# madsjulia/GeostatInversion.jl

Measured on AMD Instinct MI355X. Metric: randSVD GB/s + top-k singular-value rel-err, n=1e6 rank=256, higher is better.
Workload: dtype f64

## Files before the change

### geostatinversion.jl_amd/build.py

```python
import os
import shutil
import subprocess
import sys
from concurrent.futures import ThreadPoolExecutor

HERE = os.path.dirname(os.path.abspath(__file__))
CSRC = os.path.join(HERE, "csrc")
OBJ = os.path.join(HERE, "build")
LIB = os.path.join(HERE, "libgsi_hip.so")
SOURCES = ["gemm_f64.hip", "gemm_f64_gen1.hip", "syrk_f64.hip", "panel_lu_leaf.hip", "panel_lu_blocks.hip", "panel_lu_streamed.hip", "panel_lu_sharded.hip", "panel_qr.hip", "cholqr.hip", "lowrank_power.hip", "jacobi_svd.hip", "misc.hip", "lsqr_dev.hip", "block_cg.hip", "block_pcg.hip", "block_slq.hip", "pivoted_chol.hip", "pointcov_gemm.hip", "fft_cov.hip", "fft_gridcov_plan.hip", "fftrf_sample.hip", "fftrf_interp.hip", "interp_adjoint.hip", "gridcov_sample.hip","pcga_forward.hip", "fwd_adjoint.hip", "chol_saddle.hip", "posterior_var.hip",
           "hip_backend.hip", "hip_backend_products.hip", "hip_backend_sampler.hip", "hip_backend_panels.hip", "hip_backend_lowrank.hip", "hip_backend_pcga.hip",
           "hip_comm.hip", "pipeline.cpp", "solvers.cpp", "pcga.cpp", "api.cpp"]
HEADERS = ["backend.hpp", "hip_backend.hpp", "hip_backend_impl.hpp", "hip_common.hpp", "panel_lu_dev.hpp", "pipeline.hpp", "solvers.hpp", "pcga.hpp", "lsqr_state.hpp", "cg_state.hpp", "block_cg_host.hpp", "slq_state.hpp", "pchol_state.hpp", "pivoted_chol_host.hpp", "pointcov.hpp", "pointcov_gen.hpp", "host_staging.hpp", "gemm_f64_kernel.inc.hpp", "fft_line.hpp", "jacobi_sched.hpp", "fwd_plan.hpp", "fwd_adjoint_plan.hpp", "fwd_adjoint_host.hpp", "fftrf_points.hpp", "interp_adjoint_plan.hpp", "saddle_host.hpp", "posterior_host.hpp", "../../include/gsi_hip.h"]
CXXFLAGS = ["-O3", "-std=c++17", "-fPIC", "--offload-arch=gfx950", "-Wall", "-Wno-unused-function",
            "-Wno-unused-result", "-Wno-unused-value"]
RESOURCE_FLAG = "-Rpass-analysis=kernel-resource-usage"
_RES_KEYS = {"TotalSGPRs": "sgprs", "VGPRs": "vgprs", "AGPRs": "agprs", "ScratchSize [bytes/lane]": "scratch_bytes_per_lane",
             "Occupancy [waves/SIMD]": "occupancy_waves_per_simd", "SGPRs Spill": "sgpr_spills", "VGPRs Spill": "vgpr_spills",
             "LDS Size [bytes/block]": "lds_bytes_per_block", "Dynamic Stack": "dynamic_stack"}


def parse_resource_remarks(text):
    out, cur = {}, None
    for line in text.splitlines():
        if "remark:" not in line or "[-Rpass-analysis=kernel-resource-usage]" not in line:
            continue
        body = line.split("remark:", 1)[1].replace("[-Rpass-analysis=kernel-resource-usage]", "").strip()
        if ":" not in body:
            continue
        key, val = [x.strip() for x in body.rsplit(":", 1)]
        if key == "Function Name":
            cur = out.setdefault(val, {})
        elif cur is not None and key in _RES_KEYS:
            cur[_RES_KEYS[key]] = (val == "True") if key == "Dynamic Stack" else int(val)
    return out

# ... 82 lines not shown
```

### geostatinversion.jl_amd/context.py

```python
import ctypes as C

import numpy as np

from . import _lib as L


class Context:

    def __init__(self, device=0, lib=None):
        self.lib = lib or L.load()
        h = C.c_void_p()
        L.check(self.lib.gsi_ctx_create(C.byref(h), int(device)), self.lib)
        self.h = h
        self.device = int(device)
        self._children = []

    def close(self):
        if getattr(self, "h", None):
            for ch in list(self._children):
                ch.close()
            self.lib.gsi_ctx_destroy(self.h)
            self.h = None

    def __del__(self):
# ... 34 lines not shown
        row0 = min(r * pad, m)
        return row0, min(pad, m - row0)

    def profile(self, on=True):
        L.check(self.lib.gsi_ctx_profile(self.h, int(on)), self.lib)

    def phase_reset(self):
        L.check(self.lib.gsi_ctx_phase_reset(self.h), self.lib)

    def phase_times(self):
        ms = (C.c_double * len(L.PHASES))()
        cnt = (C.c_int64 * len(L.PHASES))()
        L.check(self.lib.gsi_ctx_phase_times(self.h, ms, cnt), self.lib)
        return {name: (ms[i], cnt[i]) for i, name in enumerate(L.PHASES)}

    def counters(self):
        out = (C.c_int64 * 4)()
        L.check(self.lib.gsi_ctx_counters(self.h, out), self.lib)
        return {"cholqr2": out[0], "householder": out[1], "jacobi_sweeps": out[2], "scholqr3": out[3]}

    LU_FORMS = ["none", "replicated", "per-step", "persistent-1hop", "persistent-2hop", "persistent-ov"]

    def path_info(self):
        n = 20
        out = (C.c_int64 * n)()
        L.check(self.lib.gsi_ctx_path_info(self.h, out, n), self.lib)
        forms = {self.LU_FORMS[f]: int(out[6 + f]) for f in range(1, 6) if out[6 + f]}
        return {"lu_form": self.LU_FORMS[out[0]] if 0 <= out[0] < 6 else int(out[0]), "lu_forms_run": forms,
                "lu_selftest_mask": int(out[1]), "collectives": int(out[2]), "n_ranks_seen": int(out[3]),
                "lu_timeouts": int(out[4]), "lu_timeouts_recovered": int(out[5]), "svd_sweep_cap_hits": int(out[12]),
                "lowrank_tails": int(out[13]), "lowrank_power_steps": int(out[14]), "lowrank_power_declines": int(out[15]),
                "lowrank_split_lus": int(out[16]), "lowrank_split_declines": int(out[17]),
                "lowrank_tail_overlaps": int(out[18]), "lowrank_tail_series_rounds": int(out[19])}

    def release_cache(self):
        L.check(self.lib.gsi_ctx_release_cache(self.h), self.lib)

    def device_bytes(self):
        b = C.c_int64()
        L.check(self.lib.gsi_ctx_device_bytes(self.h, C.byref(b)), self.lib)
        return b.value


class _Handle:
    _destroy = None

    def __init__(self, ctx, h):
        self.ctx, self.h = ctx, h
        ctx._children.append(self)

    def close(self):
        if getattr(self, "h", None):
            getattr(self.ctx.lib, self._destroy)(self.h)
            self.h = None
            if self in self.ctx._children:
                self.ctx._children.remove(self)
# ... 190 lines not shown
```

### geostatinversion.jl_amd/csrc/api.cpp

```cpp
#include <cmath>
#include <cstdlib>
#include <cstring>
#include <memory>
#include <new>
#include <string>
#include <vector>
#include "../../include/gsi_hip.h"
#include "pcga.hpp"
#include "solvers.hpp"
#include "pointcov.hpp"
#include "fftrf_points.hpp"
#include "cg_state.hpp"

using namespace gsi;

struct gsi_ctx {
  Context c;
};
struct gsi_op {
  Operator op;
};
struct gsi_mat {
  gsi_ctx* ctx;
  Buf buf;
// ... 178 lines not shown
  });
}

int gsi_ctx_path_info(gsi_ctx* ctx, int64_t* out, int64_t n_out) {
  return guarded([&] {
    REQUIRE(ctx && out && n_out >= 1, "bad argument");
    Context& c = ctx->c;
    int64_t v[GSI_PATH_INFO_COUNT] = {0};
    v[GSI_PATH_LU_FORM_LAST] = c.lu_form_last;
    v[GSI_PATH_LU_SELFTEST_MASK] = c.lus_mr_selftest;
    v[GSI_PATH_COLLECTIVES] = c.comm ? c.comm->ncollectives : 0;
    v[GSI_PATH_RANKS_SEEN] = c.ranks_seen;
    v[GSI_PATH_LU_TIMEOUTS] = c.be->lu_timeouts();
    v[GSI_PATH_LU_TIMEOUTS_RECOVERED] = c.lu_timeouts_recovered;
    for (int f = 0; f < (int)Context::LU_FORMS; ++f) v[GSI_PATH_LU_FORM_COUNTS + f] = c.lu_form_count[f];
    v[GSI_PATH_SVD_CAP_HITS] = c.be->svd_cap_hits();
    v[GSI_PATH_LOWRANK_TAILS] = c.lowrank_tails;
    v[GSI_PATH_LOWRANK_POWER_STEPS] = c.lowrank_power_steps;
    v[GSI_PATH_LOWRANK_POWER_DECLINES] = c.lowrank_power_declines;
    v[GSI_PATH_LOWRANK_SPLIT_LUS] = c.lowrank_split_lus;
    v[GSI_PATH_LOWRANK_SPLIT_DECLINES] = c.lowrank_split_declines;
    v[GSI_PATH_LOWRANK_TAIL_OVERLAPS] = c.be->lowrank_tail_overlaps();
    v[GSI_PATH_LOWRANK_TAIL_SERIES_ROUNDS] = c.be->lowrank_tail_series_rounds();
    for (int64_t i = 0; i < n_out; ++i) out[i] = i < GSI_PATH_INFO_COUNT ? v[i] : 0;
  });
}

int gsi_ctx_pinned_copy_rate(gsi_ctx* ctx, int64_t bytes, double* h2d_gbs, double* d2h_gbs) {
  return guarded([&] {
    REQUIRE(ctx && h2d_gbs && d2h_gbs, "NULL argument");
    REQUIRE(bytes >= 0 && bytes <= ((int64_t)64 << 30), "bad size");
    ctx->c.be->pinned_copy_rate(bytes, h2d_gbs, d2h_gbs);
  });
}

int gsi_ctx_rank(gsi_ctx* ctx, int* rank, int* nranks) {
  return guarded([&] {
    REQUIRE(ctx, "ctx is NULL");
    if (rank) *rank = ctx->c.rank();
    if (nranks) *nranks = ctx->c.nranks();
  });
}

int gsi_op_dense(gsi_ctx* ctx, gsi_op** op, const double* A_rows, int64_t m, int64_t n, int64_t lda,
                 int64_t row0, int64_t m_local) {
  return guarded([&] {
// ... 937 lines not shown
int gsi_gemm(gsi_ctx* ctx, int trans, int64_t m, int64_t l, int64_t k, double alpha, const double* A,
             int64_t lda, const double* B, int64_t ldb, double* C, int64_t ldc) {
  return guarded([&] {
    REQUIRE(ctx && A && B && C, "NULL argument");
    REQUIRE(m >= 1 && l >= 1 && k >= 1, "bad shape");
    const int64_t ar = trans ? k : m, ac = trans ? m : k;
    REQUIRE(lda >= ar && ldb >= k && ldc >= m, "leading dimension too small");
    Backend* be = ctx->c.be.get();
    Buf Ad(be, (size_t)ar * ac), Bd(be, (size_t)k * l), Cd(be, (size_t)m * l);
    be->upload2d(Ad.p, ar, A, lda, ar, ac);
    be->upload2d(Bd.p, k, B, ldb, k, l);
    if (trans) be->gemm_tn(m, l, k, alpha, Ad.p, ar, Bd.p, k, 0.0, Cd.p, m);
    else be->gemm_nn(m, l, k, alpha, Ad.p, ar, Bd.p, k, 0.0, Cd.p, m);
    be->download2d(C, ldc, Cd.p, m, m, l);
    check_async_errors(ctx->c);
  });
}

int gsi_gemm_view(gsi_ctx* ctx, int form, int trans, int64_t m, int64_t l, int64_t k, double alpha, double beta,
                  const double* A, int64_t lda, int64_t a_off, const double* B, int64_t ldb, int64_t b_off, double* C,
                  int64_t ldc, int64_t c_off, int64_t m_full, int64_t r0, int64_t* plan_out) {
  return guarded([&] {
    REQUIRE(ctx && A && C && plan_out, "NULL argument");
    REQUIRE(form >= 0 && form <= 3, "gemm_view: form is 0 (gemm), 1 (syrk upper), 2 (trmm upper) or 3 (NN row block)");
    REQUIRE(m >= 1 && l >= 1 && k >= 1, "bad shape");
    REQUIRE(form == 1 || B, "NULL argument");
    REQUIRE(form == 0 || (alpha == 1.0 && beta == 0.0), "gemm_view: forms 1 to 3 compute C = op(A) B (alpha 1, beta 0)");
    REQUIRE(form == 0 || !trans, "gemm_view: trans belongs to form 0");
    REQUIRE(form != 1 || m == l, "gemm_view: form 1 is the l x l product A'A (m == l)");
    REQUIRE(form != 3 || (r0 >= 0 && r0 + m <= m_full), "gemm_view: row block outside the full product");
    const bool tn = trans || form == 1;
    const int64_t ar = (form == 3) ? m_full : (tn ? k : m), ac = tn ? m : k;
    const int64_t crows = (form == 3) ? m_full : m;
    REQUIRE(lda >= ar && ldc >= crows && (form == 1 || ldb >= k), "leading dimension too small");
    REQUIRE(a_off >= 0 && b_off >= 0 && c_off >= 0, "negative offset");
    Backend* be = ctx->c.be.get();
    const size_t na = (size_t)a_off + (size_t)lda * (size_t)ac, nc = (size_t)c_off + (size_t)ldc * (size_t)l;
    const size_t nb = (form == 1) ? 1 : (size_t)b_off + (size_t)ldb * (size_t)l;
    Buf Ad(be, na), Bd(be, nb), Cd(be, nc);
    be->fill_bytes(Ad.p, 0xFF, na);
    be->fill_bytes(Bd.p, 0xFF, nb);
    be->upload2d(Ad.p + a_off, lda, A, ar, ar, ac);
    if (form != 1) be->upload2d(Bd.p + b_off, ldb, B, k, k, l);
    be->upload2d(Cd.p, (int64_t)nc, C, (int64_t)nc, (int64_t)nc, 1);
    be->gemm_view(form, trans != 0, m, l, k, alpha, Ad.p + a_off, lda, Bd.p + b_off, ldb, beta, Cd.p + c_off, ldc, m_full, r0,
                  plan_out);
    be->download2d(C, (int64_t)nc, Cd.p, (int64_t)nc, (int64_t)nc, 1);
    check_async_errors(ctx->c);
  });
}

// ... 699 lines not shown
```

### geostatinversion.jl_amd/csrc/backend.hpp

```cpp
#pragma once
#include <cstddef>
#include <cstdint>
#include <stdexcept>
#include <string>

namespace gsi {

struct Error : std::runtime_error {
  int code;
  Error(int c, const std::string& msg) : std::runtime_error(msg), code(c) {}
};

enum Phase : int {
  PH_GEMM_N = 0, PH_GEMM_T = 1, PH_LU = 2, PH_QR = 3, PH_SVD = 4, PH_SMALL_GEMM = 5,
  PH_COMM = 6, PH_OTHER = 7, PH_COMM_WAIT = 8, PH_COUNT = 9
};

struct FwdProduct {
  int64_t nobs = 0, n = 0, nnz = 0, nseg = 0, maxlen = 0;
  const int64_t* segptr = nullptr;
  const int64_t* rowseg = nullptr;
  const int32_t* colidx = nullptr;
  const double* vals = nullptr;
  const double* w = nullptr;
// ... 125 lines not shown
  virtual bool lus_mr_swaps_done() { return false; }
  virtual void lus_swap_pack(const double*, int64_t, int64_t, int64_t, int64_t, int64_t, int, double*) {}
  virtual void lus_swap_apply(double*, int64_t, int64_t, int64_t, int64_t, int64_t, int, const double*) {}
  virtual void qr_thinQ(double* Y, int64_t m, int64_t l, int64_t ld, double* R, bool replicated = false) = 0;
  virtual bool qr_thinQ_deferred(const double* Y, int64_t m, int64_t l, int64_t ld, const double** Q1, int64_t* ldq1,
                                 double* X2) { (void)Y; (void)m; (void)l; (void)ld; (void)Q1; (void)ldq1; (void)X2; return false; }
  virtual bool svd_tall_fused(const double*, int64_t, int64_t, int64_t, int64_t, double*, int64_t, double*, const double* Xr = nullptr) {
    (void)Xr;
    return false;
  }
  virtual bool sample_gram(const double* S, int64_t ld, int64_t n, int64_t N, double* G) {
    (void)S; (void)ld; (void)n; (void)N; (void)G;
    return false;
  }
  virtual bool lowrank_tail(const double* S, int64_t lds, int64_t n, int64_t N, const double* G, const double* T, int64_t l,
                            int64_t K, double c, double* Z, int64_t ldz, double* Sv, double* scratch = nullptr,
                            size_t scratch_doubles = 0) {
    (void)S; (void)lds; (void)n; (void)N; (void)G; (void)T; (void)l; (void)K; (void)c; (void)Z; (void)ldz; (void)Sv;
    (void)scratch; (void)scratch_doubles;
    return false;
  }
  virtual int64_t lowrank_tail_overlaps() { return 0; }
  virtual int64_t lowrank_tail_series_rounds() { return 0; }
  virtual void cq_gram_round_view(double* Gm, int64_t l, double* X, bool check, int32_t* out2, double* norm_out) {
    (void)Gm; (void)l; (void)X; (void)check; (void)out2; (void)norm_out;
    throw Error(1 , "cq_gram_round: not available on this backend");
  }
  virtual bool lowrank_power_step(const double* S, int64_t lds, int64_t n, int64_t N, const double* G, const double* T,
                                  const int32_t* ipiv, const double* L, int64_t ldl, int64_t l, double c, double* T_next) {
    (void)S; (void)lds; (void)n; (void)N; (void)G; (void)T; (void)ipiv; (void)L; (void)ldl; (void)l; (void)c; (void)T_next;
    return false;
  }
  virtual bool lowrank_split_ok(int64_t n, int64_t N, int64_t l, int64_t l1) {
    (void)n; (void)N; (void)l; (void)l1;
    return false;
  }
  virtual void lowrank_split_schur(const double* S, int64_t lds, int64_t n, int64_t N, const double* T, const int32_t* ipiv1,
                                   const double* P, int64_t ldp, int64_t l, int64_t l1, double c, double* Tt) {
    (void)S; (void)lds; (void)n; (void)N; (void)T; (void)ipiv1; (void)P; (void)ldp; (void)l; (void)l1; (void)c; (void)Tt;
    throw Error(1 , "lowrank_split_schur: not available on this backend");
  }
  virtual void lowrank_split_rows(double* P, int64_t ldp, int64_t n, int64_t l, int64_t l1) {
    (void)P; (void)ldp; (void)n; (void)l; (void)l1;
    throw Error(1 , "lowrank_split_rows: not available on this backend");
  }
  virtual void lowrank_split_join(double* P, int64_t ldp, int64_t n, int64_t l, int64_t l1, const int32_t* ipiv2,
// ... 228 lines not shown
```

### geostatinversion.jl_amd/csrc/hip_backend_impl.hpp

```cpp
#pragma once
#include <map>
#include <memory>
#include <mutex>
#include <set>
#include <string>
#include <vector>
#include "hip_backend.hpp"
#include "hip_common.hpp"
#include "host_staging.hpp"
#include "fftrf_points.hpp"

namespace gsi {

struct DevBuf {
  void* p = nullptr;
  size_t bytes = 0;
  bool pooled = false;
};

struct Carve {
  size_t total = 0;
  static constexpr size_t up8(size_t x) { return (x + 7) & ~(size_t)7; }
  size_t take(size_t count) { const size_t o = total; total += up8(count); return o; }
  size_t packed(size_t count) { const size_t o = total; total += count; return o; }
// ... 66 lines not shown
  void* upload2d_begin(double* dst, int64_t ldd, const double* host, int64_t ldh, int64_t rows, int64_t cols,
                       int64_t block_rows) override;
  void upload2d_wait_block(void* handle, int64_t b) override;
  void upload2d_end(void* handle) override;
  void pinned_copy_rate(int64_t bytes, double* h2d_gbs, double* d2h_gbs) override;
  void copy2d(double* dst, int64_t ldd, const double* src, int64_t lds, int64_t rows, int64_t cols) override;
  void fill_zero(double* p, size_t count) override;
  void fill_bytes(double* p, int byte, size_t count) override;
  void sync() override;
  void forgive_lost_coresidency() override;
  bool retryable_failure() override;
  int take_error(std::string* msg) override;
  void profile(bool on) override { prof_ = on; }
  void phase_begin(Phase p) override;
  void phase_end(Phase) override { phase_end_counted(true); }
  void phase_end_more(Phase) override { phase_end_counted(false); }
  void phase_reset() override;
  void phase_times(double* ms, int64_t* counts) override;
  void counters(int64_t* out4) override;
  int64_t lu_timeouts() override { return n_lu_timeouts_; }
  int64_t svd_cap_hits() override { return n_svd_cap_hits_; }
  int64_t lowrank_tail_overlaps() override { return n_tail_overlaps_; }
  int64_t lowrank_tail_series_rounds() override { return n_tail_series_rounds_; }
  void set_ranks_sharing_device(int n) override { ranks_sharing_device_ = n; }

  void gemm_nn(int64_t m, int64_t l, int64_t k, double alpha, const double* A, int64_t lda, const double* B,
               int64_t ldb, double beta, double* C, int64_t ldc) override;
  void gemm_nn_rowblock(int64_t m_full, int64_t r0, int64_t mb, int64_t l, int64_t k, const double* A, int64_t lda,
                        const double* B, int64_t ldb, double* C, int64_t ldc) override;
  void gemm_tn(int64_t m, int64_t l, int64_t k, double alpha, const double* A, int64_t lda, const double* B,
               int64_t ldb, double beta, double* C, int64_t ldc) override;
  void gemm_view(int form, bool trans, int64_t m, int64_t l, int64_t k, double alpha, const double* A, int64_t lda,
                 const double* B, int64_t ldb, double beta, double* C, int64_t ldc, int64_t m_full, int64_t r0,
                 int64_t* plan8) override;
  void gemm_nn_gridcov(int64_t m, int64_t l, int64_t k, const double* tab, int64_t nx, int64_t ny, int64_t roff,
                       int64_t koff, const double* B, int64_t ldb, double* C, int64_t ldc) override;
  void gemm_nn_pointcov(int64_t m, int64_t l, int64_t k, const double* pts, int d, int kind, double ell, double sigma2,
                        double nugget, int64_t roff, int64_t koff, const double* B, int64_t ldb, double* C,
                        int64_t ldc) override;
  void* fftcov_create(const int64_t N[3], double beta, int fftrf) override;
  void* fftcov_create_lags(const int64_t N[3], int kind, const double ell[3], double theta, double sigma2, double nugget,
                           const double* table, const double* table_mirror) override;
  void fftcov_destroy(void* plan) override;
  void fftcov_apply(void* plan, int64_t l, const double* X, int64_t ldx, double* Y, int64_t ldy) override;
  void center_rows(double* S, int64_t n, int64_t N, int64_t ld) override;
  void randn(double* p, size_t count, uint64_t seed) override;
// ... 123 lines not shown
                       double* x, bool* singular) override;
  int basis_quadform(const void* Z, int zbits, int64_t n, int64_t ldz, int64_t K, const double* W, int64_t ldw, int64_t ncols,
                     bool upper, const double* u, double* a, double* q, double* t) override;
  int scale_rows(int64_t m, int64_t c, const double* d, const double* src, int64_t lds, double* dst, int64_t ldd) override;

 private:
  void trim_pool(int64_t keep_bytes);
  void free_ws(DevBuf& b);
  void collect_garbage();
  void trim(DevBuf& b);
  void grow(DevBuf& b, size_t bytes);
  GemmWs gemm_ws(size_t doubles);
  HostStager* stager();
  static size_t stage_min_bytes();
  bool staged(bool h2d, double* dev, int64_t ldd, double* host, int64_t ldh, int64_t rows, int64_t cols);
  void drain_side() { if (st2_) (void)hipStreamSynchronize(st2_); }
  hipStream_t side_stream();
  int32_t read_flag(int slot);
  void check_launch(const char* what);
  void phase_end_counted(bool counted);
  hipEvent_t get_event();

  void fits_ws(const char* who, const char* form, size_t need, const GemmWs& ws, int64_t m, int64_t l, int64_t k);
  void gemm(const char* who, const GemmWs& ws, bool trans, int64_t m, int64_t l, int64_t k, double alpha, const double* A,
            int64_t lda, const double* B, int64_t ldb, double beta, double* C, int64_t ldc, hipk::GemmPlan* plan = nullptr);
  void gemm_rowblock(const char* who, const GemmWs& ws, int64_t m_full, int64_t r0, int64_t mb, int64_t l, int64_t k,
                     const double* A, int64_t lda, const double* B, int64_t ldb, double* C, int64_t ldc,
                     hipk::GemmPlan* plan = nullptr);
  void gemm_syrk_upper(const char* who, const GemmWs& ws, int64_t l, int64_t k, const double* A, int64_t lda, double* C,
                       int64_t ldc, hipk::GemmPlan* plan = nullptr);
  void gemm_trmm_upper(const char* who, const GemmWs& ws, int64_t m, int64_t l, int64_t k, const double* A, int64_t lda,
                       const double* B, int64_t ldb, double* C, int64_t ldc, hipk::GemmPlan* plan = nullptr);
  std::unique_ptr<FftCov> fftcov_new_plan(const int64_t N[3], int fftrf, bool* reembed, int* dims);
  void fft_rotate_apply(Scratch& buf, int64_t cur[3], int64_t& tot, int d, int64_t rows_out, int64_t period, FftFactor f);
  void fftcov_lags_to_spectrum(Scratch& bufh, int64_t cur[3], int64_t& tot, const FftCov* p, int d, bool sine);
  static size_t points_plan_doubles(const FftrfPointsPlan& plan);
  void upload_points_plan(const FftrfPointsPlan& plan, double* d);
  void interp_batch(const FftrfPointsPlan& plan, const double* dplan, const double* V, int64_t v_fs, int nb, double* dst,
                    int64_t ldd);
  void fftrf_batches(double* dst, int64_t ldd, int64_t row0, int64_t nloc, int64_t nf, int ndims, const int64_t* N, double k0,
                     double dk, double beta, const double* phi, int64_t ldphi, uint64_t seed, int64_t field0,
                     const FftrfPointsPlan* at);

  void lu_L_impl(double* Y, int64_t m, int64_t l, int64_t ld, int32_t* ipiv_host, int32_t** ipiv_dev_out);
  bool lu2_resident_ok() const;
  bool lu2_takes(int64_t m, hipk::Lu2Work* w);
// ... 16 lines not shown
  DevBuf ws_gemm_, ws_lu_, ws_split_, ws_qr_, ws_svd_, ws_blas2_, ws_lus_, ws_svdf_, ws_qr_hh_;
  DevBuf* const ws_all_[9] = {&ws_gemm_, &ws_lu_, &ws_split_, &ws_qr_, &ws_svd_, &ws_blas2_, &ws_lus_, &ws_svdf_, &ws_qr_hh_};
  std::mutex mu_;
  std::vector<DevBuf> sizes_;
  std::vector<DevBuf> pool_;
  std::vector<void*> garbage_;
  size_t garbage_bytes_ = 0;
  int64_t in_use_ = 0, pooled_ = 0;

  std::unique_ptr<HostStager> stager_;
  bool stager_failed_ = false;
  hipEvent_t ev_stage_ = nullptr;

  bool prof_ = false;
  Rec cur_{};
  std::vector<Rec> records_;
  std::vector<hipEvent_t> ev_pool_;
  double acc_ms_[PH_COUNT] = {0};
  int64_t acc_n_[PH_COUNT] = {0};
  int last_svd_sweeps_ = 0;
  int64_t n_svd_cap_hits_ = 0;
  int64_t n_cholqr_ = 0, n_householder_ = 0, n_scholqr3_ = 0;
  int64_t n_tail_overlaps_ = 0;
  int64_t n_tail_series_rounds_ = 0;

  std::map<std::pair<int64_t, bool>, int> skip_tier1_by_height_;

  std::map<int, int> lu2_resident_;
  bool lu2_lost_ = false, lu2_retry_ = false;
  int lu2_ov_resident_ = -1;

  int mr_force_ = 0;
  unsigned long long* mr_recs_ = nullptr;
  unsigned long long* mr_peer_[hipk::LU2_MAX_RANKS] = {nullptr};
  Comm* mr_comm_ = nullptr;
  uint32_t mr_epoch_ = 0;
  bool mr_disabled_ = false, mr_peer_swaps_ = true;
  bool mr_share_tried_ = false, mr_in_flight_ = false;
  int64_t mr_gen_ = 0, n_lu_timeouts_ = 0;
  std::string mr_reason_, mr_why_disabled_;
  std::set<int64_t> mr_warm_;
  hipk::Lu2MrWork mr_work_{};
  int64_t lus_part_col_ = -1, lus_part_mloc_ = 0;
  const double* lus_part_Y_ = nullptr;

  void* pin_power_ = nullptr;
// ... 4 lines not shown
```

### geostatinversion.jl_amd/csrc/hip_backend_products.hip

```cpp
#include <algorithm>
#include <cmath>
#include <cstdlib>
#include <cstring>
#include "hip_backend_impl.hpp"
#include "interp_adjoint_plan.hpp"

namespace gsi {

void HipBackend::fits_ws(const char* who, const char* form, size_t need, const GemmWs& ws, int64_t m, int64_t l, int64_t k) {
  if (need <= ws.doubles) return;
  throw Error(GSI_ERR_INTERNAL, std::string(who) + ": the " + form + " product " + std::to_string(m) + " x " + std::to_string(l) +
                                    " (K = " + std::to_string(k) + ") needs a workspace of " + std::to_string(need) +
                                    " doubles and was given " + std::to_string(ws.doubles));
}
void HipBackend::gemm(const char* who, const GemmWs& ws, bool trans, int64_t m, int64_t l, int64_t k, double alpha,
                      const double* A, int64_t lda, const double* B, int64_t ldb, double beta, double* C, int64_t ldc,
                      hipk::GemmPlan* plan) {
  fits_ws(who, trans ? "A'B" : "AB", hipk::gemm_workspace_doubles(m, l, k), ws, m, l, k);
  hipk::gemm_f64(st_, trans, m, l, k, alpha, A, lda, B, ldb, beta, C, ldc, ws.p, plan);
}
void HipBackend::gemm_rowblock(const char* who, const GemmWs& ws, int64_t m_full, int64_t r0, int64_t mb, int64_t l, int64_t k,
                               const double* A, int64_t lda, const double* B, int64_t ldb, double* C, int64_t ldc,
                               hipk::GemmPlan* plan) {
  fits_ws(who, "row-block", hipk::gemm_rowblock_workspace_doubles(m_full, mb, l, k), ws, mb, l, k);
  hipk::gemm_f64_nn_rowblock(st_, m_full, r0, mb, l, k, A, lda, B, ldb, C, ldc, ws.p, plan);
}
void HipBackend::gemm_syrk_upper(const char* who, const GemmWs& ws, int64_t l, int64_t k, const double* A, int64_t lda,
                                 double* C, int64_t ldc, hipk::GemmPlan* plan) {
  fits_ws(who, "A'A", hipk::gemm_syrk_workspace_doubles(l, k), ws, l, l, k);
  hipk::gemm_f64_syrk_upper(st_, l, k, A, lda, C, ldc, ws.p, plan);
}
void HipBackend::gemm_trmm_upper(const char* who, const GemmWs& ws, int64_t m, int64_t l, int64_t k, const double* A,
                                 int64_t lda, const double* B, int64_t ldb, double* C, int64_t ldc, hipk::GemmPlan* plan) {
  fits_ws(who, "A triu(B)", hipk::gemm_workspace_doubles(m, l, k), ws, m, l, k);
  hipk::gemm_f64_trmm_upper(st_, m, l, k, A, lda, B, ldb, C, ldc, ws.p, plan);
}

void HipBackend::gemm_nn(int64_t m, int64_t l, int64_t k, double alpha, const double* A, int64_t lda, const double* B,
                         int64_t ldb, double beta, double* C, int64_t ldc) {
  bind();
// ... 2 lines not shown
  check_launch("gemm_nn");
}
void HipBackend::gemm_nn_rowblock(int64_t m_full, int64_t r0, int64_t mb, int64_t l, int64_t k, const double* A, int64_t lda,
                                  const double* B, int64_t ldb, double* C, int64_t ldc) {
  bind();
  const GemmWs ws = gemm_ws(hipk::gemm_rowblock_workspace_doubles(m_full, mb, l, k));
  gemm_rowblock("gemm_nn_rowblock", ws, m_full, r0, mb, l, k, A, lda, B, ldb, C, ldc);
  check_launch("gemm_nn_rowblock");
}
void HipBackend::gemm_tn(int64_t m, int64_t l, int64_t k, double alpha, const double* A, int64_t lda, const double* B,
                         int64_t ldb, double beta, double* C, int64_t ldc) {
  bind();
  const GemmWs ws = gemm_ws(hipk::gemm_workspace_doubles(m, l, k));
  gemm("gemm_tn", ws, true, m, l, k, alpha, A, lda, B, ldb, beta, C, ldc);
  check_launch("gemm_tn");
}
void HipBackend::gemm_view(int form, bool trans, int64_t m, int64_t l, int64_t k, double alpha, const double* A, int64_t lda,
                           const double* B, int64_t ldb, double beta, double* C, int64_t ldc, int64_t m_full, int64_t r0,
                           int64_t* plan8) {
  bind();
  hipk::GemmPlan p = {0, 0, 0, 0, 0, 0, 0, 0};
  if (form == 0) {
    const GemmWs ws = gemm_ws(hipk::gemm_workspace_doubles(m, l, k));
    gemm("gemm_view", ws, trans, m, l, k, alpha, A, lda, B, ldb, beta, C, ldc, &p);
  } else if (form == 1) {
    const GemmWs ws = gemm_ws(hipk::gemm_syrk_workspace_doubles(l, k));
    gemm_syrk_upper("gemm_view", ws, l, k, A, lda, C, ldc, &p);
  } else if (form == 2) {
    const GemmWs ws = gemm_ws(hipk::gemm_workspace_doubles(m, l, k));
    gemm_trmm_upper("gemm_view", ws, m, l, k, A, lda, B, ldb, C, ldc, &p);
  } else {
    const GemmWs ws = gemm_ws(hipk::gemm_rowblock_workspace_doubles(m_full, m, l, k));
    gemm_rowblock("gemm_view", ws, m_full, r0, m, l, k, A, lda, B, ldb, C, ldc, &p);
  }
  check_launch("gemm_view");
  const int64_t out[8] = {p.nt, p.nchunks, p.xmode, p.wide, p.nsplit, p.persistent, p.grid_x, p.active};
  for (int i = 0; i < 8; ++i) plan8[i] = out[i];
}
void HipBackend::gemm_nn_gridcov(int64_t m, int64_t l, int64_t k, const double* tab, int64_t nx, int64_t ny, int64_t roff,
                                 int64_t koff, const double* B, int64_t ldb, double* C, int64_t ldc) {
  bind();
  double* ws = gemm_ws(hipk::gemm_workspace_doubles(m, l, k)).p;
  hipk::gemm_f64_gridcov(st_, m, l, k, tab, nx, ny, roff, koff, B, ldb, C, ldc, ws);
  check_launch("gemm_nn_gridcov");
}

void HipBackend::gemm_nn_pointcov(int64_t m, int64_t l, int64_t k, const double* pts, int d, int kind, double ell, double sigma2,
// ... 307 lines not shown
```

### geostatinversion.jl_amd/csrc/hip_common.hpp

```cpp
#pragma once
#include <hip/hip_runtime.h>
#include <atomic>
#include <cstdint>
#include <cstddef>
#include "pointcov.hpp"

namespace gsi { struct FwdProduct; struct FwdAdjoint; }

namespace gsi { namespace hipk {

inline bool first_use_on_this_device(std::atomic<uint64_t>& mask) {
  int dev = 0;
  if (hipGetDevice(&dev) != hipSuccess || dev < 0 || dev > 63) return true;
  const uint64_t bit = (uint64_t)1 << dev;
  return (mask.fetch_or(bit, std::memory_order_acq_rel) & bit) == 0;
}

struct GemmPlan { int64_t nt, nchunks, xmode, wide, nsplit, persistent, grid_x, active; };
size_t gemm_workspace_doubles(int64_t M, int64_t L, int64_t K);
void gemm_f64(hipStream_t st, bool transA, int64_t M, int64_t L, int64_t K, double alpha, const double* A,
              int64_t lda, const double* B, int64_t ldb, double beta, double* C, int64_t ldc, double* ws,
              GemmPlan* plan = nullptr);
bool gemm_f64_nn_capped(hipStream_t st, int64_t M, int64_t L, int64_t K, const double* A, int64_t lda, const double* B,
                        int64_t ldb, double* C, int64_t ldc, int max_grid, bool query_only = false, GemmPlan* plan = nullptr);
// ... 3 lines not shown
                          GemmPlan* plan = nullptr);
size_t gemm_syrk_workspace_doubles(int64_t l, int64_t m);
size_t syrk_upper_workspace_doubles(int64_t l, int64_t m);
bool syrk_full_from_upper(hipStream_t st, int64_t l, int64_t m, const double* Y, int64_t ld, double* G, int64_t ldg, double* ws);
bool trmm_upper_tall(hipStream_t st, int64_t m, int64_t l, const double* A, int64_t lda, const double* X, int64_t ldx, double* C,
                     int64_t ldc);
void gemm_f64_syrk_upper(hipStream_t st, int64_t l, int64_t m, const double* A, int64_t lda, double* C, int64_t ldc,
                         double* ws, GemmPlan* plan = nullptr);
void gemm_f64_trmm_upper(hipStream_t st, int64_t M, int64_t L, int64_t K, const double* A, int64_t lda, const double* B,
                         int64_t ldb, double* C, int64_t ldc, double* ws, GemmPlan* plan = nullptr);
void gemm_f64_gridcov(hipStream_t st, int64_t M, int64_t L, int64_t K, const double* tab, int64_t nx, int64_t ny,
                      int64_t roff, int64_t koff, const double* B, int64_t ldb, double* C, int64_t ldc, double* ws);

void gemm_f64_pointcov(hipStream_t st, int64_t M, int64_t L, int64_t K, const double* pts4, int64_t npts, int d, int kind,
                       double sigma2, double nugget, int64_t roff, int64_t koff, const double* B, int64_t ldb, double* C,
                       int64_t ldc, double* ws, double* xpack);
double pointcov_point_scale(int kind, double inv_ell);
bool gemm_f64_pointcov_wide(hipStream_t st, int64_t M, int64_t L, int64_t K, const double* pts4, int64_t npts, int d, int kind,
                            double sigma2, double nugget, int64_t roff, int64_t koff, const double* B, int64_t ldb, double* C,
                            int64_t ldc, double* ws, double* xpack);
size_t gemm_pointcov_workspace_doubles(int64_t M, int64_t L, int64_t K);
size_t gemm_pointcov_pack_doubles(int64_t M, int64_t L, int64_t K);
int gemm_choose_split(int64_t nwg, int64_t K);
void gemm_splitk_reduce(hipStream_t st, int64_t M, int64_t L, int nsplit, const double* slabs, double* C, int64_t ldc);
void pointcov_pad_points(hipStream_t st, const double* pts, int d, int64_t n, double scale, double* out4);
int64_t fft_embed_size(int64_t N);
size_t fft_plan_doubles(const int64_t M[3]);
void fft_spectrum(hipStream_t st, double* lam, double* part64, const int64_t M[3], double beta, int fftrf);
void fft_cos_matrix(hipStream_t st, double* out, int64_t rows, int64_t cols, int64_t period, bool weighted);
void fft_lines_layout(hipStream_t st, const double* nat, double* out, const int64_t M[3]);
void fft_spectrum_natural(hipStream_t st, double* lam, const int64_t M[3], double beta, int fftrf);
void fft_finish_plan(hipStream_t st, double* lam, double* part64, const int64_t M[3]);
void fft_plan_twiddles(hipStream_t st, double* lam, const int64_t M[3]);
void fft_lag_table(hipStream_t st, double* cp, double* cm, const int64_t N[3], int kind, const double inv_ell[3], double cs,
                   double sn, double sigma2);
void fft_even_odd_split(hipStream_t st, double* cp, double* cm, int64_t total);
void fft_sin_matrix(hipStream_t st, double* out, int64_t rows, int64_t cols, int64_t period);
void fft_subtract(hipStream_t st, double* a, const double* b, int64_t total);
void fft_finish_plan_lags(hipStream_t st, double* lam, const int64_t M[3], double nugget);
void fft_cov_apply(hipStream_t st, const int64_t N[3], const int64_t M[3], const double* lam, double2* W, int nb_max,
                   int64_t l, const double* X, int64_t ldx, double* Y, int64_t ldy);

struct FftrfGeom { int d; int64_t A[3], L[3], P[3]; int blue[3]; int64_t Mtot, n; };
void fftrf_geometry(int ndims, const int64_t* N, FftrfGeom* g);
size_t fftrf_plan_doubles(const FftrfGeom& g);
size_t fftrf_field_doubles(const FftrfGeom& g);
// ... 253 lines not shown
```

### include/gsi_hip.h

```cpp
#ifndef GSI_HIP_H
#define GSI_HIP_H

#include <stdint.h>

#ifdef __cplusplus
extern "C" {
#endif

#define GSI_VERSION 100

#define GSI_OK 0
#define GSI_ERR_ARG 1
#define GSI_ERR_NEG_ITERS 2
#define GSI_ERR_SINGULAR 3
#define GSI_ERR_HIP 4
#define GSI_ERR_RCCL 5
#define GSI_ERR_OOM 6
#define GSI_ERR_NOT_POSDEF 7
#define GSI_ERR_INTERNAL 8

typedef struct gsi_ctx gsi_ctx;
typedef struct gsi_op gsi_op;
typedef struct gsi_mat gsi_mat;

// ... 219 lines not shown
#define GSI_PHASE_OTHER 7
#define GSI_PHASE_COMM_WAIT 8
#define GSI_NUM_PHASES 9
int gsi_ctx_profile(gsi_ctx* ctx, int enable);
int gsi_ctx_phase_reset(gsi_ctx* ctx);
int gsi_ctx_phase_times(gsi_ctx* ctx, double* ms_out ,
                        int64_t* count_out );
int gsi_ctx_counters(gsi_ctx* ctx, int64_t* out4);
#define GSI_PATH_LU_FORM_LAST 0
#define GSI_PATH_LU_SELFTEST_MASK 1
#define GSI_PATH_COLLECTIVES 2
#define GSI_PATH_RANKS_SEEN 3
#define GSI_PATH_LU_TIMEOUTS 4
#define GSI_PATH_LU_TIMEOUTS_RECOVERED 5
#define GSI_PATH_LU_FORM_COUNTS 6
#define GSI_PATH_SVD_CAP_HITS 12
#define GSI_PATH_LOWRANK_TAILS 13
#define GSI_PATH_LOWRANK_POWER_STEPS 14
#define GSI_PATH_LOWRANK_POWER_DECLINES 15
#define GSI_PATH_LOWRANK_SPLIT_LUS 16
#define GSI_PATH_LOWRANK_SPLIT_DECLINES 17
#define GSI_PATH_LOWRANK_TAIL_OVERLAPS 18
#define GSI_PATH_LOWRANK_TAIL_SERIES_ROUNDS 19
#define GSI_PATH_INFO_COUNT 20
int gsi_ctx_path_info(gsi_ctx* ctx, int64_t* out, int64_t n_out);
int gsi_ctx_pinned_copy_rate(gsi_ctx* ctx, int64_t bytes, double* h2d_gbs, double* d2h_gbs);
int gsi_ctx_release_cache(gsi_ctx* ctx);
int gsi_ctx_device_bytes(gsi_ctx* ctx, int64_t* bytes);

#ifdef __cplusplus
}
#endif
#endif
```

Before: 1777.

## Route small GEMMs to a dedicated 32x32 MFMA f64 kernel

Adds a small-shape f64 GEMM kernel that uses 32x32 output tiles, a four-deep register prefetch ring and double-buffered LDS, with in-kernel split-K accumulation in place of a separate reduce pass. HipBackend::gemm now sends shapes with K up to 1280 and bounded m*l*k to this kernel by default, so the many small products in the randomized SVD (Gram and small projections) get more workgroups, no workspace and no reduce launch. The kernel does not split K across workgroups; it accumulates the split ranges serially inside one block, so long-K shapes may lose parallelism. A counter and a gemm_view form 4 are exposed for testing.

```diff
diff --git a/geostatinversion.jl_amd/build.py b/geostatinversion.jl_amd/build.py
--- a/geostatinversion.jl_amd/build.py
+++ b/geostatinversion.jl_amd/build.py
@@ -8,10 +8,10 @@
 CSRC = os.path.join(HERE, "csrc")
 OBJ = os.path.join(HERE, "build")
 LIB = os.path.join(HERE, "libgsi_hip.so")
-SOURCES = ["gemm_f64.hip", "gemm_f64_gen1.hip", "syrk_f64.hip", "panel_lu_leaf.hip", "panel_lu_blocks.hip", "panel_lu_streamed.hip", "panel_lu_sharded.hip", "panel_qr.hip", "cholqr.hip", "lowrank_power.hip", "jacobi_svd.hip", "misc.hip", "lsqr_dev.hip", "block_cg.hip", "block_pcg.hip", "block_slq.hip", "pivoted_chol.hip", "pointcov_gemm.hip", "fft_cov.hip", "fft_gridcov_plan.hip", "fftrf_sample.hip", "fftrf_interp.hip", "interp_adjoint.hip", "gridcov_sample.hip","pcga_forward.hip", "fwd_adjoint.hip", "chol_saddle.hip", "posterior_var.hip",
+SOURCES = ["gemm_f64.hip", "gemm_f64_gen1.hip", "gemm_f64_small.hip", "syrk_f64.hip", "panel_lu_leaf.hip", "panel_lu_blocks.hip", "panel_lu_streamed.hip", "panel_lu_sharded.hip", "panel_qr.hip", "cholqr.hip", "lowrank_power.hip", "jacobi_svd.hip", "misc.hip", "lsqr_dev.hip", "block_cg.hip", "block_pcg.hip", "block_slq.hip", "pivoted_chol.hip", "pointcov_gemm.hip", "fft_cov.hip", "fft_gridcov_plan.hip", "fftrf_sample.hip", "fftrf_interp.hip", "interp_adjoint.hip", "gridcov_sample.hip","pcga_forward.hip", "fwd_adjoint.hip", "chol_saddle.hip", "posterior_var.hip",
            "hip_backend.hip", "hip_backend_products.hip", "hip_backend_sampler.hip", "hip_backend_panels.hip", "hip_backend_lowrank.hip", "hip_backend_pcga.hip",
            "hip_comm.hip", "pipeline.cpp", "solvers.cpp", "pcga.cpp", "api.cpp"]
-HEADERS = ["backend.hpp", "hip_backend.hpp", "hip_backend_impl.hpp", "hip_common.hpp", "panel_lu_dev.hpp", "pipeline.hpp", "solvers.hpp", "pcga.hpp", "lsqr_state.hpp", "cg_state.hpp", "block_cg_host.hpp", "slq_state.hpp", "pchol_state.hpp", "pivoted_chol_host.hpp", "pointcov.hpp", "pointcov_gen.hpp", "host_staging.hpp", "gemm_f64_kernel.inc.hpp", "fft_line.hpp", "jacobi_sched.hpp", "fwd_plan.hpp", "fwd_adjoint_plan.hpp", "fwd_adjoint_host.hpp", "fftrf_points.hpp", "interp_adjoint_plan.hpp", "saddle_host.hpp", "posterior_host.hpp", "../../include/gsi_hip.h"]
+HEADERS = ["backend.hpp", "hip_backend.hpp", "hip_backend_impl.hpp", "hip_common.hpp", "panel_lu_dev.hpp", "pipeline.hpp", "solvers.hpp", "pcga.hpp", "lsqr_state.hpp", "cg_state.hpp", "block_cg_host.hpp", "slq_state.hpp", "pchol_state.hpp", "pivoted_chol_host.hpp", "pointcov.hpp", "pointcov_gen.hpp", "host_staging.hpp", "gemm_f64_kernel.inc.hpp", "small_gemm_plan.hpp", "fft_line.hpp", "jacobi_sched.hpp", "fwd_plan.hpp", "fwd_adjoint_plan.hpp", "fwd_adjoint_host.hpp", "fftrf_points.hpp", "interp_adjoint_plan.hpp", "saddle_host.hpp", "posterior_host.hpp", "../../include/gsi_hip.h"]
 CXXFLAGS = ["-O3", "-std=c++17", "-fPIC", "--offload-arch=gfx950", "-Wall", "-Wno-unused-function",
             "-Wno-unused-result", "-Wno-unused-value"]
 RESOURCE_FLAG = "-Rpass-analysis=kernel-resource-usage"
diff --git a/geostatinversion.jl_amd/context.py b/geostatinversion.jl_amd/context.py
--- a/geostatinversion.jl_amd/context.py
+++ b/geostatinversion.jl_amd/context.py
@@ -80,7 +80,7 @@
     LU_FORMS = ["none", "replicated", "per-step", "persistent-1hop", "persistent-2hop", "persistent-ov"]
 
     def path_info(self):
-        n = 20
+        n = 21
         out = (C.c_int64 * n)()
         L.check(self.lib.gsi_ctx_path_info(self.h, out, n), self.lib)
         forms = {self.LU_FORMS[f]: int(out[6 + f]) for f in range(1, 6) if out[6 + f]}
@@ -89,7 +89,8 @@
                 "lu_timeouts": int(out[4]), "lu_timeouts_recovered": int(out[5]), "svd_sweep_cap_hits": int(out[12]),
                 "lowrank_tails": int(out[13]), "lowrank_power_steps": int(out[14]), "lowrank_power_declines": int(out[15]),
                 "lowrank_split_lus": int(out[16]), "lowrank_split_declines": int(out[17]),
-                "lowrank_tail_overlaps": int(out[18]), "lowrank_tail_series_rounds": int(out[19])}
+                "lowrank_tail_overlaps": int(out[18]), "lowrank_tail_series_rounds": int(out[19]),
+                "small_gemm_launches": int(out[20])}
 
     def release_cache(self):
         L.check(self.lib.gsi_ctx_release_cache(self.h), self.lib)
diff --git a/geostatinversion.jl_amd/csrc/api.cpp b/geostatinversion.jl_amd/csrc/api.cpp
--- a/geostatinversion.jl_amd/csrc/api.cpp
+++ b/geostatinversion.jl_amd/csrc/api.cpp
@@ -224,6 +224,7 @@
     v[GSI_PATH_LOWRANK_SPLIT_DECLINES] = c.lowrank_split_declines;
     v[GSI_PATH_LOWRANK_TAIL_OVERLAPS] = c.be->lowrank_tail_overlaps();
     v[GSI_PATH_LOWRANK_TAIL_SERIES_ROUNDS] = c.be->lowrank_tail_series_rounds();
+    v[GSI_PATH_SMALL_GEMMS] = c.be->small_gemm_launches();
     for (int64_t i = 0; i < n_out; ++i) out[i] = i < GSI_PATH_INFO_COUNT ? v[i] : 0;
   });
 }
@@ -1207,11 +1208,13 @@
                   int64_t ldc, int64_t c_off, int64_t m_full, int64_t r0, int64_t* plan_out) {
   return guarded([&] {
     REQUIRE(ctx && A && C && plan_out, "NULL argument");
-    REQUIRE(form >= 0 && form <= 3, "gemm_view: form is 0 (gemm), 1 (syrk upper), 2 (trmm upper) or 3 (NN row block)");
+    REQUIRE(form >= 0 && form <= 4,
+            "gemm_view: form is 0 (gemm), 1 (syrk upper), 2 (trmm upper), 3 (NN row block) or 4 (gemm on the small-shape kernel)");
     REQUIRE(m >= 1 && l >= 1 && k >= 1, "bad shape");
     REQUIRE(form == 1 || B, "NULL argument");
-    REQUIRE(form == 0 || (alpha == 1.0 && beta == 0.0), "gemm_view: forms 1 to 3 compute C = op(A) B (alpha 1, beta 0)");
-    REQUIRE(form == 0 || !trans, "gemm_view: trans belongs to form 0");
+    const bool plain = form == 0 || form == 4;
+    REQUIRE(plain || (alpha == 1.0 && beta == 0.0), "gemm_view: forms 1 to 3 compute C = op(A) B (alpha 1, beta 0)");
+    REQUIRE(plain || !trans, "gemm_view: trans belongs to forms 0 and 4");
     REQUIRE(form != 1 || m == l, "gemm_view: form 1 is the l x l product A'A (m == l)");
     REQUIRE(form != 3 || (r0 >= 0 && r0 + m <= m_full), "gemm_view: row block outside the full product");
     const bool tn = trans || form == 1;
diff --git a/geostatinversion.jl_amd/csrc/backend.hpp b/geostatinversion.jl_amd/csrc/backend.hpp
--- a/geostatinversion.jl_amd/csrc/backend.hpp
+++ b/geostatinversion.jl_amd/csrc/backend.hpp
@@ -171,6 +171,7 @@
   }
   virtual int64_t lowrank_tail_overlaps() { return 0; }
   virtual int64_t lowrank_tail_series_rounds() { return 0; }
+  virtual int64_t small_gemm_launches() { return 0; }
   virtual void cq_gram_round_view(double* Gm, int64_t l, double* X, bool check, int32_t* out2, double* norm_out) {
     (void)Gm; (void)l; (void)X; (void)check; (void)out2; (void)norm_out;
     throw Error(1 , "cq_gram_round: not available on this backend");
diff --git a/geostatinversion.jl_amd/csrc/gemm_f64_small.hip b/geostatinversion.jl_amd/csrc/gemm_f64_small.hip
--- /dev/null
+++ b/geostatinversion.jl_amd/csrc/gemm_f64_small.hip
@@ -0,0 +1,179 @@
+#include <hip/hip_runtime.h>
+#include <cstdint>
+#include "hip_common.hpp"
+
+namespace gsi { namespace hipk {
+
+namespace {
+typedef double sg_double4 __attribute__((ext_vector_type(4)));
+constexpr int SG_TM = 32, SG_TL = 32;
+constexpr int SG_BK = 32;
+constexpr int SG_BKP = SG_BK + 2;
+constexpr int SG_THREADS = 256;
+constexpr int SG_SETS = 4;
+constexpr int SG_PER = SG_TM * SG_BK / SG_THREADS;
+constexpr int SG_IMG = SG_TM * SG_BKP;
+static_assert(SG_TM == SG_TL && SG_PER * SG_THREADS == SG_TM * SG_BK, "tile does not divide over the threads");
+static_assert(SG_SETS % 2 == 0, "the LDS buffer of a tile is the parity of its register set");
+
+__device__ __forceinline__ uint32_t sg_lt_mask(int a, int b) { return (uint32_t)((a - b) >> 31); }
+__device__ __forceinline__ double sg_and(double v, uint32_t m) {
+  const uint64_t bits = (uint64_t)__double_as_longlong(v);
+  const uint32_t lo = (uint32_t)bits & m, hi = (uint32_t)(bits >> 32) & m;
+  return __longlong_as_double((long long)(((uint64_t)hi << 32) | lo));
+}
+
+template <bool TRANS_A, bool FULL>
+__device__ __forceinline__ void sg_tiles(double* smem, int M, int L, int K, const double* __restrict__ A, int64_t lda,
+                                         const double* __restrict__ B, int64_t ldb, int r0, int c0, int tiles_per_range, int ns_eff,
+                                         sg_double4& acc, sg_double4& tot) {
+  const int tid = threadIdx.x;
+  const int lane = tid & 63, wave = tid >> 6;
+  const int rh = wave & 1, ch = wave >> 1;
+  const int jl = lane & 15, kk = lane >> 4;
+  const int ntot = (K + SG_BK - 1) / SG_BK;
+  const int lo = tid & 31, hi = tid >> 5;
+  double ra[SG_SETS][SG_PER], rb[SG_SETS][SG_PER];
+
+  uint32_t offa[SG_PER], offb[SG_PER];
+#pragma unroll
+  for (int it = 0; it < SG_PER; ++it) {
+    offb[it] = 8u * ((uint32_t)lo + (uint32_t)(hi + 8 * it) * (uint32_t)ldb);
+    offa[it] = 8u * ((uint32_t)lo + (uint32_t)(hi + 8 * it) * (uint32_t)lda);
+  }
+  const char* const Abase = reinterpret_cast<const char*>(TRANS_A ? A + (int64_t)r0 * lda : A + r0);
+  const char* const Bbase = reinterpret_cast<const char*>(B + (int64_t)c0 * ldb);
+  const int64_t a_tile = 8 * (TRANS_A ? (int64_t)SG_BK : (int64_t)SG_BK * lda);
+  auto fetch = [&](int j, int set) __attribute__((always_inline)) {
+    if (FULL) {
+      const int jt = (j < ntot) ? j : ntot - 1;
+      const char* Ab = Abase + (int64_t)jt * a_tile;
+      const char* Bb = Bbase + (int64_t)jt * (8 * SG_BK);
+#pragma unroll
+      for (int it = 0; it < SG_PER; ++it) {
+        rb[set][it] = *reinterpret_cast<const double*>(Bb + offb[it]);
+        ra[set][it] = *reinterpret_cast<const double*>(Ab + offa[it]);
+      }
+      return;
+    }
+    const int jj = (j < ntot) ? j : ntot - 1;
+    const int k0 = jj * SG_BK;
+#pragma unroll
+    for (int it = 0; it < SG_PER; ++it) {
+      const int h = hi + 8 * it;
+      const int kb = min(k0 + lo, K - 1), cb = min(c0 + h, L - 1);
+      const int ka = min(TRANS_A ? k0 + lo : k0 + h, K - 1), ra_ = min(TRANS_A ? r0 + h : r0 + lo, M - 1);
+      rb[set][it] = B[(int64_t)kb + (int64_t)cb * ldb];
+      ra[set][it] = TRANS_A ? A[(int64_t)ka + (int64_t)ra_ * lda] : A[(int64_t)ra_ + (int64_t)ka * lda];
+    }
+  };
+  auto stage = [&](int j, int buf, int set) __attribute__((always_inline)) {
+    double* a_s = smem + buf * 2 * SG_IMG;
+    double* b_s = a_s + SG_IMG;
+    const int k0 = j * SG_BK;
+#pragma unroll
+    for (int it = 0; it < SG_PER; ++it) {
+      const int h = hi + 8 * it;
+      double vb = rb[set][it], va = ra[set][it];
+      if (!FULL) {
+        vb = sg_and(vb, sg_lt_mask(k0 + lo, K) & sg_lt_mask(c0 + h, L));
+        va = TRANS_A ? sg_and(va, sg_lt_mask(k0 + lo, K) & sg_lt_mask(r0 + h, M))
+                     : sg_and(va, sg_lt_mask(k0 + h, K) & sg_lt_mask(r0 + lo, M));
+      }
+      b_s[h * SG_BKP + lo] = vb;
+      if (TRANS_A) a_s[h * SG_BKP + lo] = va;
+      else a_s[lo * SG_BKP + h] = va;
+    }
+  };
+
+  int range_end = tiles_per_range;
+#pragma unroll
+  for (int u = 0; u < SG_SETS; ++u) fetch(u, u);
+  stage(0, 0, 0);
+  fetch(SG_SETS, 0);
+  __syncthreads();
+
+  for (int jb = 0; jb < ntot; jb += SG_SETS) {
+#pragma unroll
+    for (int u = 0; u < SG_SETS; ++u) {
+      const int j = jb + u;
+      const int cur = u & 1;
+      const int nset = (u + 1) % SG_SETS;
+      const double* a_s = smem + cur * 2 * SG_IMG + (16 * rh + jl) * SG_BKP + kk;
+      const double* b_s = smem + cur * 2 * SG_IMG + SG_IMG + (16 * ch + jl) * SG_BKP + kk;
+      double fa[SG_BK / 4], fb[SG_BK / 4];
+#pragma unroll
+      for (int s = 0; s < SG_BK / 4; ++s) { fa[s] = a_s[4 * s]; fb[s] = b_s[4 * s]; }
+      stage(j + 1, cur ^ 1, nset);
+      fetch(j + 1 + SG_SETS, nset);
+      if (j < ntot) {
+#pragma unroll
+        for (int s = 0; s < SG_BK / 4; ++s) acc = __builtin_amdgcn_mfma_f64_16x16x4f64(fb[s], fa[s], acc, 0, 0, 0);
+        if (ns_eff > 1 && (j + 1 == range_end || j + 1 == ntot)) {
+#pragma unroll
+          for (int reg = 0; reg < 4; ++reg) tot[reg] += acc[reg];
+          acc = (sg_double4){0.0, 0.0, 0.0, 0.0};
+          range_end += tiles_per_range;
+        }
+      }
+      __syncthreads();
+    }
+  }
+}
+}
+
+template <bool TRANS_A>
+__global__ __launch_bounds__(SG_THREADS, 2) void gemm_f64_small_kernel(
+    int M, int L, int K, const double* __restrict__ A, int64_t lda, const double* __restrict__ B, int64_t ldb,
+    double* __restrict__ C, int64_t ldc, double alpha, double beta, int tiles_per_range, int ns_eff, int tiles_m, int near_ld) {
+  __shared__ double smem[2 * 2 * SG_IMG];
+  const int tm = (int)blockIdx.x % tiles_m, tl = (int)blockIdx.x / tiles_m;
+  const int r0 = tm * SG_TM;
+  const int c0 = tl * SG_TL;
+  sg_double4 acc = {0.0, 0.0, 0.0, 0.0};
+  sg_double4 tot = {0.0, 0.0, 0.0, 0.0};
+  if (r0 + SG_TM <= M && c0 + SG_TL <= L && K % SG_BK == 0 && near_ld)
+    sg_tiles<TRANS_A, true>(smem, M, L, K, A, lda, B, ldb, r0, c0, tiles_per_range, ns_eff, acc, tot);
+  else
+    sg_tiles<TRANS_A, false>(smem, M, L, K, A, lda, B, ldb, r0, c0, tiles_per_range, ns_eff, acc, tot);
+
+  const int lane = threadIdx.x & 63, wave = threadIdx.x >> 6;
+  const int rh = wave & 1, ch = wave >> 1, jl = lane & 15, kk = lane >> 4;
+  const int row = r0 + 16 * rh + jl;
+  if (row < M) {
+#pragma unroll
+    for (int reg = 0; reg < 4; ++reg) {
+      const int col = c0 + 16 * ch + kk + 4 * reg;
+      if (col < L) {
+        double* p = C + ((int64_t)row + (int64_t)col * ldc);
+        if (ns_eff > 1) {
+          const double s = tot[reg];
+          double v = alpha * s;
+          if (beta != 0.0) v += beta * *p;
+          *p = v;
+        } else {
+          double v = alpha * acc[reg];
+          if (beta != 0.0) v += beta * *p;
+          *p = v;
+        }
+      }
+    }
+  }
+}
+
+void gemm_f64_small(hipStream_t st, bool transA, int64_t M, int64_t L, int64_t K, double alpha, const double* A, int64_t lda,
+                    const double* B, int64_t ldb, double beta, double* C, int64_t ldc, int64_t kchunk, int ns_eff, GemmPlan* plan) {
+  const int tiles_m = (int)((M + SG_TM - 1) / SG_TM), tiles_l = (int)((L + SG_TL - 1) / SG_TL);
+  const dim3 grid((unsigned)(tiles_m * tiles_l));
+  if (plan != nullptr) *plan = {SG_TL / 16, tiles_l, 3, 0, ns_eff, 0, (int64_t)grid.x, (int64_t)grid.x};
+  const int tpr = (int)(kchunk / SG_BK);
+  const int near_ld = (lda < ((int64_t)1 << 23) && ldb < ((int64_t)1 << 23)) ? 1 : 0;
+  if (transA)
+    hipLaunchKernelGGL((gemm_f64_small_kernel<true>), grid, dim3(SG_THREADS), 0, st, (int)M, (int)L, (int)K, A, lda, B, ldb, C, ldc,
+                       alpha, beta, tpr, ns_eff, tiles_m, near_ld);
+  else
+    hipLaunchKernelGGL((gemm_f64_small_kernel<false>), grid, dim3(SG_THREADS), 0, st, (int)M, (int)L, (int)K, A, lda, B, ldb, C, ldc,
+                       alpha, beta, tpr, ns_eff, tiles_m, near_ld);
+}
+
+}}
diff --git a/geostatinversion.jl_amd/csrc/hip_backend_impl.hpp b/geostatinversion.jl_amd/csrc/hip_backend_impl.hpp
--- a/geostatinversion.jl_amd/csrc/hip_backend_impl.hpp
+++ b/geostatinversion.jl_amd/csrc/hip_backend_impl.hpp
@@ -112,6 +112,7 @@
   int64_t svd_cap_hits() override { return n_svd_cap_hits_; }
   int64_t lowrank_tail_overlaps() override { return n_tail_overlaps_; }
   int64_t lowrank_tail_series_rounds() override { return n_tail_series_rounds_; }
+  int64_t small_gemm_launches() override { return n_small_gemms_; }
   void set_ranks_sharing_device(int n) override { ranks_sharing_device_ = n; }
 
   void gemm_nn(int64_t m, int64_t l, int64_t k, double alpha, const double* A, int64_t lda, const double* B,
@@ -281,6 +282,8 @@
   hipEvent_t get_event();
 
   void fits_ws(const char* who, const char* form, size_t need, const GemmWs& ws, int64_t m, int64_t l, int64_t k);
+  bool gemm_small(bool trans, int64_t m, int64_t l, int64_t k, double alpha, const double* A, int64_t lda, const double* B,
+                  int64_t ldb, double beta, double* C, int64_t ldc, bool forced, hipk::GemmPlan* plan);
   void gemm(const char* who, const GemmWs& ws, bool trans, int64_t m, int64_t l, int64_t k, double alpha, const double* A,
             int64_t lda, const double* B, int64_t ldb, double beta, double* C, int64_t ldc, hipk::GemmPlan* plan = nullptr);
   void gemm_rowblock(const char* who, const GemmWs& ws, int64_t m_full, int64_t r0, int64_t mb, int64_t l, int64_t k,
@@ -343,6 +346,7 @@
   int64_t n_svd_cap_hits_ = 0;
   int64_t n_cholqr_ = 0, n_householder_ = 0, n_scholqr3_ = 0;
   int64_t n_tail_overlaps_ = 0;
+  int64_t n_small_gemms_ = 0;
   int64_t n_tail_series_rounds_ = 0;
 
   std::map<std::pair<int64_t, bool>, int> skip_tier1_by_height_;
diff --git a/geostatinversion.jl_amd/csrc/hip_backend_products.hip b/geostatinversion.jl_amd/csrc/hip_backend_products.hip
--- a/geostatinversion.jl_amd/csrc/hip_backend_products.hip
+++ b/geostatinversion.jl_amd/csrc/hip_backend_products.hip
@@ -4,6 +4,7 @@
 #include <cstring>
 #include "hip_backend_impl.hpp"
 #include "interp_adjoint_plan.hpp"
+#include "small_gemm_plan.hpp"
 
 namespace gsi {
 
@@ -13,9 +14,23 @@
                                     " (K = " + std::to_string(k) + ") needs a workspace of " + std::to_string(need) +
                                     " doubles and was given " + std::to_string(ws.doubles));
 }
+bool HipBackend::gemm_small(bool trans, int64_t m, int64_t l, int64_t k, double alpha, const double* A, int64_t lda,
+                            const double* B, int64_t ldb, double beta, double* C, int64_t ldc, bool forced, hipk::GemmPlan* plan) {
+  static const bool routing_on = !(getenv("GSI_SMALL_GEMM") != nullptr && getenv("GSI_SMALL_GEMM")[0] == '0');
+  if (!forced && !routing_on) return false;
+  if (m < 1 || l < 1 || k < 1) return false;
+  const smallgemm::Call call = {m, l, k, false, 0, false, false};
+  const int ns = hipk::gemm_choose_split(smallgemm::tall_active_tiles(m, l), k);
+  if (!(forced ? smallgemm::small_gemm_hard_ok(call, ns) : smallgemm::small_gemm_routes(call, ns))) return false;
+  const smallgemm::Partition p = smallgemm::partition_for(m, l, k, ns);
+  hipk::gemm_f64_small(st_, trans, m, l, k, alpha, A, lda, B, ldb, beta, C, ldc, p.kchunk, p.ns_eff, plan);
+  if (!forced) ++n_small_gemms_;
+  return true;
+}
 void HipBackend::gemm(const char* who, const GemmWs& ws, bool trans, int64_t m, int64_t l, int64_t k, double alpha,
                       const double* A, int64_t lda, const double* B, int64_t ldb, double beta, double* C, int64_t ldc,
                       hipk::GemmPlan* plan) {
+  if (gemm_small(trans, m, l, k, alpha, A, lda, B, ldb, beta, C, ldc, false, plan)) return;
   fits_ws(who, trans ? "A'B" : "AB", hipk::gemm_workspace_doubles(m, l, k), ws, m, l, k);
   hipk::gemm_f64(st_, trans, m, l, k, alpha, A, lda, B, ldb, beta, C, ldc, ws.p, plan);
 }
@@ -64,7 +79,11 @@
   hipk::GemmPlan p = {0, 0, 0, 0, 0, 0, 0, 0};
   if (form == 0) {
     const GemmWs ws = gemm_ws(hipk::gemm_workspace_doubles(m, l, k));
-    gemm("gemm_view", ws, trans, m, l, k, alpha, A, lda, B, ldb, beta, C, ldc, &p);
+    fits_ws("gemm_view", trans ? "A'B" : "AB", hipk::gemm_workspace_doubles(m, l, k), ws, m, l, k);
+    hipk::gemm_f64(st_, trans, m, l, k, alpha, A, lda, B, ldb, beta, C, ldc, ws.p, &p);
+  } else if (form == 4) {
+    if (!gemm_small(trans, m, l, k, alpha, A, lda, B, ldb, beta, C, ldc, true, &p))
+      throw Error(GSI_ERR_ARG, "gemm_view: the small-shape kernel does not take this shape (small_gemm_plan.hpp: hard limits)");
   } else if (form == 1) {
     const GemmWs ws = gemm_ws(hipk::gemm_syrk_workspace_doubles(l, k));
     gemm_syrk_upper("gemm_view", ws, l, k, A, lda, C, ldc, &p);
diff --git a/geostatinversion.jl_amd/csrc/hip_common.hpp b/geostatinversion.jl_amd/csrc/hip_common.hpp
--- a/geostatinversion.jl_amd/csrc/hip_common.hpp
+++ b/geostatinversion.jl_amd/csrc/hip_common.hpp
@@ -49,6 +49,9 @@
 size_t gemm_pointcov_workspace_doubles(int64_t M, int64_t L, int64_t K);
 size_t gemm_pointcov_pack_doubles(int64_t M, int64_t L, int64_t K);
 int gemm_choose_split(int64_t nwg, int64_t K);
+void gemm_f64_small(hipStream_t st, bool transA, int64_t M, int64_t L, int64_t K, double alpha, const double* A, int64_t lda,
+                    const double* B, int64_t ldb, double beta, double* C, int64_t ldc, int64_t kchunk, int ns_eff,
+                    GemmPlan* plan = nullptr);
 void gemm_splitk_reduce(hipStream_t st, int64_t M, int64_t L, int nsplit, const double* slabs, double* C, int64_t ldc);
 void pointcov_pad_points(hipStream_t st, const double* pts, int d, int64_t n, double scale, double* out4);
 int64_t fft_embed_size(int64_t N);
diff --git a/geostatinversion.jl_amd/csrc/small_gemm_plan.hpp b/geostatinversion.jl_amd/csrc/small_gemm_plan.hpp
--- /dev/null
+++ b/geostatinversion.jl_amd/csrc/small_gemm_plan.hpp
@@ -0,0 +1,70 @@
+#pragma once
+#include <cstdint>
+
+namespace gsi { namespace smallgemm {
+
+constexpr int64_t TALL_BMT = 128, TALL_NTMAX = 10, TALL_BK = 32, TALL_CUS = 256;
+constexpr int64_t TILE_M = 32, TILE_L = 32;
+
+constexpr int64_t MAX_M = 16384, MAX_L = 16384, MAX_K = 65536, MAX_SPLITS = 256;
+constexpr int64_t ROUTE_MAX_K = 1280;
+constexpr int64_t ROUTE_MAX_MLK = (int64_t)1 << 29;
+
+struct Call {
+  int64_t m, l, k;
+  bool generated;
+  int tri;
+  bool capped;
+  bool rowblock;
+};
+struct Partition {
+  int64_t active;
+  int nsplit;
+  int64_t kchunk;
+  int ns_eff;
+};
+
+inline int tall_choose_split(int64_t nwg, int64_t K) {
+  if (K < 8 * TALL_BK || nwg >= 16 * TALL_CUS) return 1;
+  int64_t maxs = K / (4 * TALL_BK);
+  if (maxs > 256) maxs = 256;
+  int best = 1;
+  double best_cost = (double)((nwg + TALL_CUS - 1) / TALL_CUS);
+  for (int64_t s = 2; s <= maxs; ++s) {
+    const double cost = (double)((nwg * s + TALL_CUS - 1) / TALL_CUS) / (double)s * (1.0 + 0.004 * (double)s);
+    if (cost < 0.97 * best_cost) { best = (int)s; best_cost = cost; }
+  }
+  return best;
+}
+inline int64_t tall_active_tiles(int64_t M, int64_t L) {
+  const int64_t tiles = (L + 15) / 16, nchunks = (tiles + TALL_NTMAX - 1) / TALL_NTMAX;
+  return ((M + TALL_BMT - 1) / TALL_BMT) * nchunks;
+}
+inline Partition partition_for(int64_t M, int64_t L, int64_t K, int nsplit) {
+  Partition p;
+  p.active = tall_active_tiles(M, L);
+  p.nsplit = nsplit;
+  int64_t kchunk = (K + nsplit - 1) / nsplit;
+  kchunk = ((kchunk + TALL_BK - 1) / TALL_BK) * TALL_BK;
+  if (kchunk == 0) kchunk = TALL_BK;
+  p.kchunk = kchunk;
+  p.ns_eff = (K > 0) ? (int)((K + kchunk - 1) / kchunk) : 1;
+  return p;
+}
+inline Partition small_gemm_partition(int64_t M, int64_t L, int64_t K) {
+  return partition_for(M, L, K, K > 0 ? tall_choose_split(tall_active_tiles(M, L), K) : 1);
+}
+
+inline bool small_gemm_hard_ok(const Call& c, int chooser_nsplit) {
+  if (c.generated || c.tri != 0 || c.capped || c.rowblock) return false;
+  if (c.m < 1 || c.l < 1 || c.k < 1 || chooser_nsplit < 1) return false;
+  if (c.m > MAX_M || c.l > MAX_L || c.k > MAX_K) return false;
+  return partition_for(c.m, c.l, c.k, chooser_nsplit).ns_eff <= MAX_SPLITS;
+}
+inline bool small_gemm_routes(const Call& c, int chooser_nsplit) {
+  if (!small_gemm_hard_ok(c, chooser_nsplit)) return false;
+  if (c.k > ROUTE_MAX_K) return false;
+  return c.m * c.l <= ROUTE_MAX_MLK / c.k;
+}
+
+}}
diff --git a/include/gsi_hip.h b/include/gsi_hip.h
--- a/include/gsi_hip.h
+++ b/include/gsi_hip.h
@@ -265,7 +265,8 @@
 #define GSI_PATH_LOWRANK_SPLIT_DECLINES 17
 #define GSI_PATH_LOWRANK_TAIL_OVERLAPS 18
 #define GSI_PATH_LOWRANK_TAIL_SERIES_ROUNDS 19
-#define GSI_PATH_INFO_COUNT 20
+#define GSI_PATH_SMALL_GEMMS 20
+#define GSI_PATH_INFO_COUNT 21
 int gsi_ctx_path_info(gsi_ctx* ctx, int64_t* out, int64_t n_out);
 int gsi_ctx_pinned_copy_rate(gsi_ctx* ctx, int64_t bytes, double* h2d_gbs, double* d2h_gbs);
 int gsi_ctx_release_cache(gsi_ctx* ctx);
```

Result: no change. 1790 (median of 6 runs) (+0.7%).
